# CompVis/behavior-driven-video-synthesis

Hardware: AMD Instinct MI355X
Metric: frames/sec VUnet 256x256 bs=16 fwd+bwd (higher is better)
Workload: dtype f32 (operands scaled by a power of two and split into 2 fp16 terms, 3 partial products on fp16 MFMA, fp32 accumulate; weight gradients and uncovered layers: 3 bf16 terms / 6 products, fp32-input MFMA, fp32 VALU); 1 GPU; Human3.6m shape_and_pose_net VunetAlter 256x256 per-GPU bs=16 fwd+bwd, VGG19 perceptual + KL loss, fused Adam, dropout 0.05, regressor side loop off, seeded-synthetic VGG19 weights, rasterised synthetic stickmen; global_batch=16, parallelism=dp1, conv_precision=h2, hip_streams=4, hip_graph=True, graph_settle_steps=7, rccl_world_size=1, dp_backend=none

## Files before the change

behavior_driven_video_synthesis_amd/csrc/pointwise.hip:

```cpp
#include "common.h"

static inline dim3 ew_grid(int64_t n, int per_thread = 1) {
  int64_t b = (n + 256ll * per_thread - 1) / (256ll * per_thread);
  if (b > 2048) b = 2048;
  if (b < 1) b = 1;
  return dim3((unsigned)b);
}

#define EW_LOOP(i, n) \
  for (int64_t i = (int64_t)blockIdx.x * blockDim.x + threadIdx.x; i < (n); i += (int64_t)gridDim.x * blockDim.x)

__device__ __forceinline__ float block_sum_256(float v, float* red) {
  v = wave_sum(v);
  __syncthreads();
  if ((threadIdx.x & 63) == 0) red[threadIdx.x >> 6] = v;
  __syncthreads();
  return red[0] + red[1] + red[2] + red[3];
}

__device__ __forceinline__ float pool2_max(float e0, float e1, float e2, float e3) {
  const float m = fmaxf(fmaxf(e0, e1), fmaxf(e2, e3));
  return e3 != e3 ? e3 : (e2 != e2 ? e2 : (e1 != e1 ? e1 : (e0 != e0 ? e0 : m)));
}
__device__ __forceinline__ int pool2_route(float e0, float e1, float e2, float e3) {
// ... 339 lines not shown
__global__ void maxpool2_fwd_kernel(const float* __restrict__ x, float* __restrict__ y, int H, int W, int64_t n) {
  const int Ho = H >> 1, Wo = W >> 1;
  EW_LOOP(o, n) {
    const int ow = (int)(o % Wo);
    const int64_t t = o / Wo;
    const int oh = (int)(t % Ho);
    const int64_t nc = t / Ho;
    const float* r0 = x + (nc * H + 2 * oh) * W + 2 * ow;
    const float2 a = *reinterpret_cast<const float2*>(r0);
    const float2 b = *reinterpret_cast<const float2*>(r0 + W);
    y[o] = pool2_max(a.x, a.y, b.x, b.y);
  }
}
__global__ void maxpool2_bwd_kernel(const float* __restrict__ x, const float* __restrict__ y,
                                    const float* __restrict__ dy, float* __restrict__ dx, int H, int W, int64_t n,
                                    int relu_mask) {
  const int Ho = H >> 1, Wo = W >> 1;
  EW_LOOP(o, n) {
    const int ow = (int)(o % Wo);
    const int64_t t = o / Wo;
    const int oh = (int)(t % Ho);
    const int64_t nc = t / Ho;
    const int64_t i0 = (nc * H + 2 * oh) * W + 2 * ow;
    const float m = y[o];
    const float g = (relu_mask && m <= 0.f) ? 0.f : dy[o];
    const float2 a = *reinterpret_cast<const float2*>(x + i0);
    const float2 b = *reinterpret_cast<const float2*>(x + i0 + W);
    const int k = pool2_route(a.x, a.y, b.x, b.y);
    *reinterpret_cast<float2*>(dx + i0) = make_float2(k == 0 ? g : 0.f, k == 1 ? g : 0.f);
    *reinterpret_cast<float2*>(dx + i0 + W) = make_float2(k == 2 ? g : 0.f, k == 3 ? g : 0.f);
  }
}
extern "C" int vunet_maxpool2_fwd(const float* x, float* y, int32_t NC, int32_t H, int32_t W, void* st) {
  if (!x || !y || (H & 1) || (W & 1)) return VUNET_ERR_ARG;
  const int64_t n = (int64_t)NC * (H / 2) * (W / 2);
  VUNET_LAUNCH(maxpool2_fwd_kernel, ew_grid(n), dim3(256), 0, (hipStream_t)st, x, y, H, W, n);
  return vunet_check_launch();
}
__global__ void l1_pool_bwd_kernel(const float* __restrict__ a, const float* __restrict__ b, const float* __restrict__ dyp,
                                   float* __restrict__ db, float gs, const float* __restrict__ gout, int H, int W, int64_t n,
                                   float* __restrict__ amax_out, int relu_mask) {
  if (gout) gs *= gout[0];
  const int Ho = H >> 1, Wo = W >> 1;
  float vmax = 0.f;
  EW_LOOP(o, n) {
    const int ow = (int)(o % Wo);
    const int64_t t = o / Wo;
    const int oh = (int)(t % Ho);
    const int64_t nc = t / Ho;
    const int64_t i0 = (nc * H + 2 * oh) * W + 2 * ow;
    const float2 b0 = *reinterpret_cast<const float2*>(b + i0), b1 = *reinterpret_cast<const float2*>(b + i0 + W);
    const float2 a0 = *reinterpret_cast<const float2*>(a + i0), a1 = *reinterpret_cast<const float2*>(a + i0 + W);
    const float g = dyp ? dyp[o] : 0.f;
    const int k = pool2_route(b0.x, b0.y, b1.x, b1.y);
    const float bv[4] = {b0.x, b0.y, b1.x, b1.y}, av[4] = {a0.x, a0.y, a1.x, a1.y};
    float v[4];
#pragma unroll
    for (int e = 0; e < 4; ++e) {
      const float d = bv[e] - av[e];
      float r = (k == e ? g : 0.f) + (d > 0.f ? gs : (d < 0.f ? -gs : 0.f));
      if (relu_mask && bv[e] <= 0.f) r = 0.f;
      v[e] = r;
      vmax = fmaxf(vmax, fabsf(r));
    }
    *reinterpret_cast<float2*>(db + i0) = make_float2(v[0], v[1]);
    *reinterpret_cast<float2*>(db + i0 + W) = make_float2(v[2], v[3]);
  }
  if (amax_out) {
    const float m_ = wave_max(vmax);
    if ((threadIdx.x & 63) == 0)
      atomicMax(reinterpret_cast<unsigned*>(amax_out) + ((blockIdx.x * 4u + (threadIdx.x >> 6)) & 511u), __float_as_uint(m_));
  }
}
extern "C" int vunet_l1_pool_bwd(const float* a, const float* b, const float* dy_pool, float* db, float gscale,
                                 const float* gout, int32_t NC, int32_t H, int32_t W, float* amax_out, int32_t relu_mask,
                                 void* st) {
  if (!a || !b || !db || (H & 1) || (W & 1)) return VUNET_ERR_ARG;
  const int64_t n = (int64_t)NC * (H / 2) * (W / 2);
  VUNET_LAUNCH(l1_pool_bwd_kernel, ew_grid(n), dim3(256), 0, (hipStream_t)st, a, b, dy_pool, db, gscale, gout, H, W, n,
               amax_out, (int)relu_mask);
  return vunet_check_launch();
}

static int maxpool2_bwd(const float* x, const float* y, const float* dy, float* dx, int32_t NC, int32_t H, int32_t W,
                        int relu_mask, void* st) {
  if (!x || !y || !dy || !dx || (H & 1) || (W & 1)) return VUNET_ERR_ARG;
  const int64_t n = (int64_t)NC * (H / 2) * (W / 2);
  VUNET_LAUNCH(maxpool2_bwd_kernel, ew_grid(n), dim3(256), 0, (hipStream_t)st, x, y, dy, dx, H, W, n, relu_mask);
  return vunet_check_launch();
}
extern "C" int vunet_maxpool2_bwd(const float* x, const float* y, const float* dy, float* dx, int32_t NC, int32_t H,
                                  int32_t W, void* st) {
  return maxpool2_bwd(x, y, dy, dx, NC, H, W, 0, st);
}
extern "C" int vunet_maxpool2_bwd_relu(const float* x, const float* y, const float* dy, float* dx, int32_t NC, int32_t H,
                                       int32_t W, void* st) {
  return maxpool2_bwd(x, y, dy, dx, NC, H, W, 1, st);
}

__global__ __launch_bounds__(256) void instnorm_fwd_kernel(const float* __restrict__ x, float* __restrict__ y,
                                                           float* __restrict__ stats, int HW, float eps) {
  __shared__ float red[4];
  const float* xr = x + (size_t)blockIdx.x * HW;
  float* yr = y + (size_t)blockIdx.x * HW;
  float s = 0.f;
  for (int i = threadIdx.x; i < HW; i += 256) s += xr[i];
  const float mean = block_sum_256(s, red) / (float)HW;
  float v = 0.f;
  for (int i = threadIdx.x; i < HW; i += 256) { const float d = xr[i] - mean; v += d * d; }
  const float var = block_sum_256(v, red) / (float)HW;
  const float rstd = rsqrtf(var + eps);
  for (int i = threadIdx.x; i < HW; i += 256) yr[i] = (xr[i] - mean) * rstd;
  if (threadIdx.x == 0) { stats[2 * blockIdx.x] = mean; stats[2 * blockIdx.x + 1] = rstd; }
}
__global__ __launch_bounds__(256) void instnorm_bwd_kernel(const float* __restrict__ y, const float* __restrict__ dy,
                                                           const float* __restrict__ stats, float* __restrict__ dx,
                                                           int HW) {
  __shared__ float red[4];
  const size_t o = (size_t)blockIdx.x * HW;
  float s1 = 0.f, s2 = 0.f;
  for (int i = threadIdx.x; i < HW; i += 256) { const float g = dy[o + i]; s1 += g; s2 += g * y[o + i]; }
  const float m1 = block_sum_256(s1, red) / (float)HW;
  const float m2 = block_sum_256(s2, red) / (float)HW;
  const float rstd = stats[2 * blockIdx.x + 1];
  for (int i = threadIdx.x; i < HW; i += 256) dx[o + i] = rstd * (dy[o + i] - m1 - y[o + i] * m2);
}
extern "C" int vunet_instnorm_fwd(const float* x, float* y, float* stats, int32_t NC, int32_t HW, float eps, void* st) {
  if (!x || !y || !stats || NC <= 0 || HW <= 0) return VUNET_ERR_ARG;
  VUNET_LAUNCH(instnorm_fwd_kernel, dim3(NC), dim3(256), 0, (hipStream_t)st, x, y, stats, HW, eps);
  return vunet_check_launch();
}
extern "C" int vunet_instnorm_bwd(const float* y, const float* dy, const float* stats, float* dx, int32_t NC,
                                  int32_t HW, void* st) {
  if (!y || !dy || !stats || !dx) return VUNET_ERR_ARG;
  VUNET_LAUNCH(instnorm_bwd_kernel, dim3(NC), dim3(256), 0, (hipStream_t)st, y, dy, stats, dx, HW);
  return vunet_check_launch();
}

const uint32_t* g_vunet_drop_step = nullptr;

extern "C" int vunet_set_dropout_step(const uint32_t* step_dev) {
  g_vunet_drop_step = step_dev;
  return VUNET_OK;
}

int g_vunet_tune[16] = {0};

extern "C" int vunet_set_tuning(int32_t key, int32_t value) {
  if (key < 0 || key >= VUNET_TUNE_COUNT) return VUNET_ERR_ARG;
  g_vunet_tune[key] = value;
  return VUNET_OK;
}

__global__ void adam_kernel(float* __restrict__ p, const float* __restrict__ g, float* __restrict__ m,
                            float* __restrict__ v, int64_t n, float step_size, float b1, float b2, float eps,
                            float wd, float inv_sqrt_bc2, float gscale) {
  EW_LOOP(i, n) {
    float gi = g[i] * gscale;
    const float pi = p[i];
    if (wd != 0.f) gi += wd * pi;
    const float mi = b1 * m[i] + (1.f - b1) * gi;
    const float vi = b2 * v[i] + (1.f - b2) * gi * gi;
    m[i] = mi;
    v[i] = vi;
    const float denom = sqrtf(vi) * inv_sqrt_bc2 + eps;
    p[i] = pi - step_size * (mi / denom);
  }
}
extern "C" int vunet_adam_step(float* param, const float* grad, float* exp_avg, float* exp_avg_sq, int64_t n, float lr,
                               float beta1, float beta2, float eps, float weight_decay, int32_t step,
                               float grad_scale, void* st) {
  if (!param || !grad || !exp_avg || !exp_avg_sq || step < 1) return VUNET_ERR_ARG;
  const double bc1 = 1.0 - pow((double)beta1, (double)step);
  const double bc2 = 1.0 - pow((double)beta2, (double)step);
  VUNET_LAUNCH(adam_kernel, ew_grid(n), dim3(256), 0, (hipStream_t)st, param, grad, exp_avg, exp_avg_sq, n,
                     (float)(lr / bc1), beta1, beta2, eps, weight_decay, (float)(1.0 / sqrt(bc2)), grad_scale);
  return vunet_check_launch();
}

__global__ void adam_dev_kernel(float* __restrict__ p, const float* __restrict__ g, float* __restrict__ m,
                                float* __restrict__ v, int64_t n, const double* __restrict__ lr,
                                const int64_t* __restrict__ step, float b1, float b2, float eps, float wd, float gscale) {
  const double t = (double)*step;
  const double bc1 = 1.0 - pow((double)b1, t), bc2 = 1.0 - pow((double)b2, t);
  const float step_size = (float)((double)(float)*lr / bc1), inv_sqrt_bc2 = (float)(1.0 / sqrt(bc2));
  EW_LOOP(i, n) {
    float gi = g[i] * gscale;
    const float pi = p[i];
    if (wd != 0.f) gi += wd * pi;
    const float mi = b1 * m[i] + (1.f - b1) * gi;
    const float vi = b2 * v[i] + (1.f - b2) * gi * gi;
    m[i] = mi;
    v[i] = vi;
    const float denom = sqrtf(vi) * inv_sqrt_bc2 + eps;
    p[i] = pi - step_size * (mi / denom);
  }
}
extern "C" int vunet_adam_step_dev(float* param, const float* grad, float* exp_avg, float* exp_avg_sq, int64_t n,
                                   const double* lr_dev, float beta1, float beta2, float eps, float weight_decay,
                                   const int64_t* step_dev, float grad_scale, void* st) {
  if (!param || !grad || !exp_avg || !exp_avg_sq || !lr_dev || !step_dev) return VUNET_ERR_ARG;
  VUNET_LAUNCH(adam_dev_kernel, ew_grid(n), dim3(256), 0, (hipStream_t)st, param, grad, exp_avg, exp_avg_sq, n, lr_dev,
               step_dev, beta1, beta2, eps, weight_decay, grad_scale);
  return vunet_check_launch();
}

__global__ __launch_bounds__(256) void absmax_partials_kernel(const float* __restrict__ x1, int64_t n1,
                                                              const float* __restrict__ x2, int64_t n2,
                                                              float* __restrict__ out) {
  __shared__ float red[4];
  const bool second = blockIdx.x >= 512;
  const float* __restrict__ x = second ? x2 : x1;
  const int64_t n = second ? n2 : n1;
  const int b = second ? blockIdx.x - 512 : blockIdx.x;
  float m = 0.f;
  if (x) {
    const int64_t n4 = ((reinterpret_cast<uintptr_t>(x) & 15) == 0) ? n >> 2 : 0;
    const float4* __restrict__ x4 = reinterpret_cast<const float4*>(x);
    for (int64_t i = (int64_t)b * 256 + threadIdx.x; i < n4; i += 512 * 256) {
      const float4 v = x4[i];
      m = fmaxf(fmaxf(m, fmaxf(fabsf(v.x), fabsf(v.y))), fmaxf(fabsf(v.z), fabsf(v.w)));
    }
    for (int64_t i = 4 * n4 + (int64_t)b * 256 + threadIdx.x; i < n; i += 512 * 256) m = fmaxf(m, fabsf(x[i]));
  }
  m = wave_max(m);
  if ((threadIdx.x & 63) == 0) red[threadIdx.x >> 6] = m;
  __syncthreads();
  if (threadIdx.x == 0) out[blockIdx.x] = fmaxf(fmaxf(red[0], red[1]), fmaxf(red[2], red[3]));
}
extern "C" int vunet_absmax_partials(const float* x1, int64_t n1, const float* x2, int64_t n2, float* out, void* st) {
  if (!x1 || !out || n1 < 0 || n2 < 0) return VUNET_ERR_ARG;
  VUNET_LAUNCH(absmax_partials_kernel, dim3(1024), dim3(256), 0, (hipStream_t)st, x1, n1, x2, x2 ? n2 : 0, out);
  return vunet_check_launch();
}

__global__ void dropout_mask_kernel(float* mask, int64_t n, uint32_t thresh, uint32_t seed, const uint32_t* step) {
  if (step) seed += (*step) * VUNET_DROP_STEP_MUL;
  EW_LOOP(i, n) mask[i] = vunet_hash_u32((uint32_t)i + seed) >= thresh ? 1.f : 0.f;
}
extern "C" int vunet_dropout_mask(float* mask, int64_t n, float p, uint32_t seed, void* st) {
  if (!mask) return VUNET_ERR_ARG;
  const InAct a = make_inact(ACT_NONE, 0.f, p, seed);
  VUNET_LAUNCH(dropout_mask_kernel, ew_grid(n), dim3(256), 0, (hipStream_t)st, mask, n, a.thresh, seed, a.step);
  return vunet_check_launch();
}
__global__ void u8_to_unit_kernel(const uint8_t* in, float* out, int64_t n) {
  EW_LOOP(i, n) out[i] = ((float)in[i] / 255.0f) * 2.0f - 1.0f;
}
extern "C" int vunet_u8_to_unit(const uint8_t* in, float* out, int64_t n, void* st) {
  if (!in || !out) return VUNET_ERR_ARG;
  VUNET_LAUNCH(u8_to_unit_kernel, ew_grid(n), dim3(256), 0, (hipStream_t)st, in, out, n);
  return vunet_check_launch();
}

__device__ __forceinline__ void bil2_src(int o, int n, int& i0, int& i1, float& l) {
  const int i = o >> 1;
  if (o & 1) { i0 = i; l = 0.25f; }
  else if (i == 0) { i0 = 0; l = 0.f; }
  else { i0 = i - 1; l = 0.75f; }
  i1 = i0 + 1 < n ? i0 + 1 : n - 1;
}

__global__ void bilinear2x_fwd_kernel(const float* __restrict__ x, float* __restrict__ y, int64_t NC, int H, int W) {
  const int H2 = 2 * H, W2 = 2 * W;
  EW_LOOP(o, NC * H2 * W2) {
    const int ox = (int)(o % W2);
    const int64_t t = o / W2;
    const int oy = (int)(t % H2);
    const float* p = x + (t / H2) * H * W;
    int y0, y1, x0, x1;
    float ly, lx;
    bil2_src(oy, H, y0, y1, ly);
    bil2_src(ox, W, x0, x1, lx);
    const float top = (1.f - lx) * p[y0 * W + x0] + lx * p[y0 * W + x1];
    const float bot = (1.f - lx) * p[y1 * W + x0] + lx * p[y1 * W + x1];
    y[o] = (1.f - ly) * top + ly * bot;
  }
}

__device__ __forceinline__ void bil2_adj(int i, int n, int o[4], float w[4]) {
  o[0] = 2 * i - 1; w[0] = i >= 1 ? 0.25f : 0.f;
  o[1] = 2 * i;     w[1] = i == 0 ? 1.f : 0.75f;
  o[2] = 2 * i + 1; w[2] = i == n - 1 ? 1.f : 0.75f;
  o[3] = 2 * i + 2; w[3] = i <= n - 2 ? 0.25f : 0.f;
  if (o[0] < 0) o[0] = 0;
  if (o[3] > 2 * n - 1) o[3] = 2 * n - 1;
}

__global__ void bilinear2x_bwd_kernel(const float* __restrict__ dy, float* __restrict__ dx, int64_t NC, int H, int W) {
  const int W2 = 2 * W;
  EW_LOOP(e, NC * H * W) {
    const int ix = (int)(e % W);
    const int64_t t = e / W;
    const int iy = (int)(t % H);
    const float* p = dy + (t / H) * 4 * H * W;
    int oy[4], ox[4];
    float wy[4], wx[4];
    bil2_adj(iy, H, oy, wy);
    bil2_adj(ix, W, ox, wx);
    float s = 0.f;
#pragma unroll
    for (int a = 0; a < 4; ++a) {
      float r = 0.f;
#pragma unroll
      for (int b = 0; b < 4; ++b) r += wx[b] * p[oy[a] * W2 + ox[b]];
      s += wy[a] * r;
    }
    dx[e] = s;
  }
}

extern "C" int vunet_upsample_bilinear2x_fwd(const float* x, float* y, int64_t NC, int32_t H, int32_t W, void* st) {
  if (!x || !y || NC < 1 || H < 1 || W < 1) return VUNET_ERR_ARG;
  VUNET_LAUNCH(bilinear2x_fwd_kernel, ew_grid(NC * 4 * H * W), dim3(256), 0, (hipStream_t)st, x, y, NC, H, W);
  return vunet_check_launch();
}

extern "C" int vunet_upsample_bilinear2x_bwd(const float* dy, float* dx, int64_t NC, int32_t H, int32_t W, void* st) {
  if (!dy || !dx || NC < 1 || H < 1 || W < 1) return VUNET_ERR_ARG;
  VUNET_LAUNCH(bilinear2x_bwd_kernel, ew_grid(NC * H * W), dim3(256), 0, (hipStream_t)st, dy, dx, NC, H, W);
  return vunet_check_launch();
}

extern "C" int vunet_abi_version(void) { return 12; }

__global__ void crop_window_kernel(const float* __restrict__ x, float* __restrict__ y, int planes, int H, int W, int P,
                                   const int32_t* __restrict__ off, int bwd) {
  const int oy = off[0], ox = off[1];
  const int64_t n = (int64_t)planes * P * P;
  EW_LOOP(i, n) {
    const int j = (int)(i % P), r = (int)((i / P) % P);
    const int64_t pl = i / ((int64_t)P * P);
    const int64_t src = (pl * H + (oy + r)) * W + (ox + j);
    if (bwd) y[src] = x[i];
    else y[i] = x[src];
  }
}
extern "C" int vunet_crop_window(const float* x, float* y, int32_t planes, int32_t H, int32_t W, int32_t P, const int32_t* off,
                                 void* st) {
  if (!x || !y || !off || planes < 1 || P < 1 || P > H || P > W) return VUNET_ERR_ARG;
  VUNET_LAUNCH(crop_window_kernel, ew_grid((int64_t)planes * P * P), dim3(256), 0, (hipStream_t)st, x, y, planes, H, W, P, off, 0);
  return vunet_check_launch();
}
extern "C" int vunet_crop_window_bwd(const float* dy, float* dx, int32_t planes, int32_t H, int32_t W, int32_t P,
                                     const int32_t* off, void* st) {
  if (!dy || !dx || !off || planes < 1 || P < 1 || P > H || P > W) return VUNET_ERR_ARG;
  VUNET_LAUNCH(crop_window_kernel, ew_grid((int64_t)planes * P * P), dim3(256), 0, (hipStream_t)st, dy, dx, planes, H, W, P, off, 1);
  return vunet_check_launch();
}

struct LossTermPtrs {
  const float* t[VUNET_LOSS_MAX_TERMS];
};
__global__ void total_loss_kernel(LossTermPtrs a, int n, const float* __restrict__ kl, const float* __restrict__ gamma,
                                  float gamma_const, float ll_weight, int use_kl, float* __restrict__ loss,
// ... 112 lines not shown
```

behavior_driven_video_synthesis_amd/csrc/weightnorm.hip:

```cpp
#include "common.h"
#include "split_h2.h"

#define X6_SLAB_UNITS 576

struct WnArgs {
  vunet_wn_desc d;
  const float *v, *g, *bias, *gamma, *beta;
  float *wt_f, *wt_d, *scale, *shift, *invnorm;
  uint4 *wx_f, *wx_d;
  float* wmax;
  int T, Ctot, C1p, C2p, Kf, Mpad_f, Coutp2, Kd, Mpad_d;
};

__host__ __device__ __forceinline__ int x6_mtiles(int m) { return (((m + 31) / 32 + 1) + 1) & ~1; }

__device__ __forceinline__ uint32_t wn_pack2(float a, float b) {
  typedef __bf16 bf2 __attribute__((ext_vector_type(2)));
  bf2 p;
  p[0] = (__bf16)a;
  p[1] = (__bf16)b;
  return __builtin_bit_cast(uint32_t, p);
}

__device__ __forceinline__ void wn_split2(float a, float b, uint32_t& h, uint32_t& m, uint32_t& l) {
// ... 281 lines not shown
  const uint32_t nd = a.wt_d ? (uint32_t)a.Kd * (uint32_t)a.Mpad_d : 0u;
  const int T = a.T;
  for (uint32_t i = (uint32_t)start; i < nf + nd; i += (uint32_t)stride) {
    if (i < nf) {
      const int krow = (int)(i / (uint32_t)a.Mpad_f), m = (int)(i - (uint32_t)krow * (uint32_t)a.Mpad_f);
      int tap, c, cg;
      bool ok;
      const int k1 = T * a.C1p;
      if (krow < k1) { tap = krow / a.C1p; c = krow - tap * a.C1p; ok = c < a.d.C1; cg = c; }
      else { const int r = krow - k1; tap = r / a.C2p; c = r - tap * a.C2p; ok = c < a.d.C2; cg = a.d.C1 + c; }
      float w = 0.f;
      if (ok && m < a.d.Cout) w = a.scale[m] * a.v[((size_t)m * a.Ctot + cg) * T + tap];
      a.wt_f[i] = w;
    } else {
      const uint32_t e = i - nf;
      const int row = (int)(e / (uint32_t)a.Mpad_d), ci = (int)(e - (uint32_t)row * (uint32_t)a.Mpad_d);
      const int tap = row / a.Coutp2, co = row - tap * a.Coutp2;
      float w = 0.f;
      if (co < a.d.Cout && ci < a.Ctot) w = a.scale[co] * a.v[((size_t)co * a.Ctot + ci) * T + tap];
      a.wt_d[e] = w;
    }
  }
}

__global__ __launch_bounds__(64) void wn_scale_multi_kernel(const WnItemDev* __restrict__ items) {
  const WnItemDev& it = items[blockIdx.y];
  if ((int)blockIdx.x >= it.d.Cout) return;
  wn_scale_body(item_args(it), blockIdx.x, threadIdx.x);
}

constexpr int WN_TILE_LD = 145;

__device__ __forceinline__ bool wn_tiled_ok(const WnArgs& a) {
  return a.T == 9 && a.d.split == 2 && a.wx_f != nullptr && a.d.C1 % 16 == 0 && a.d.C2 % 16 == 0;
}

__device__ __forceinline__ void wn_pack_tile(const WnArgs& a, int mtile, int ch, float* tile) {
  const int tid = threadIdx.x;
  const int nch1 = a.d.C1 / 16;
  const bool second = ch >= nch1;
  const int cg0 = second ? a.d.C1 + (ch - nch1) * 16 : ch * 16;
  const int m0 = mtile * 32;
  const int ew = wn_layer_exp(a);
  const float sw = h2_pow2(ew);
  for (int e = tid; e < 32 * 144; e += 256) {
    const int r = e / 144, k = e - r * 144;
    const int co = m0 + r;
    tile[r * WN_TILE_LD + k] = co < a.d.Cout ? a.scale[co] * a.v[((size_t)co * a.Ctot + cg0) * 9 + k] : 0.f;
  }
  __syncthreads();
  {
    const int cl0 = second ? (ch - nch1) * 16 : ch * 16;
    const int krow0 = second ? 9 * a.C1p : 0, Cp = second ? a.C2p : a.C1p;
    for (int e = tid; e < 32 * 144; e += 256) {
      const int m = e & 31, q = e >> 5;
      const int ci = q & 15, tap = q >> 4;
      a.wt_f[(size_t)(krow0 + tap * Cp + cl0 + ci) * a.Mpad_f + m0 + m] = tile[m * WN_TILE_LD + ci * 9 + tap];
    }
  }
  if (a.wt_d) {
    for (int e = tid; e < 32 * 144; e += 256) {
      const int ci = e & 15, q = e >> 4;
      const int r = q & 31, tap = q >> 5;
      const int co = m0 + r;
      if (co < a.Coutp2) a.wt_d[(size_t)(tap * a.Coutp2 + co) * a.Mpad_d + cg0 + ci] = tile[r * WN_TILE_LD + ci * 9 + tap];
    }
  }
  {
    uint4* const out = a.wx_f + 1;
    const int mtp = x6_mtiles(a.d.Cout);
    if (mtile == 0 && ch == 0 && tid == 0) a.wx_f[0] = make_uint4((uint32_t)ew, 0u, 0u, 0u);
    for (int e = tid; e < 9 * 2 * 32; e += 256) {
      const int j = e & 31, half = (e >> 5) & 1, tap = e >> 6;
      const int kh = tap / 3, kw = tap - 3 * kh;
      float w[8];
#pragma unroll
      for (int c = 0; c < 8; ++c) w[c] = tile[j * WN_TILE_LD + (half * 8 + c) * 9 + tap] * sw;
      uint4 ph, pl;
      h2_split2(w[0], w[1], ph.x, pl.x);
      h2_split2(w[2], w[3], ph.y, pl.y);
      h2_split2(w[4], w[5], ph.z, pl.z);
      h2_split2(w[6], w[7], ph.w, pl.w);
      const size_t base = ((((size_t)(ch * 3 + kh) * mtp + mtile) * 3 + kw) * 2) * 64 + half * 32 + j;
      out[base] = ph;
      out[base + 64] = pl;
    }
  }
  if (a.wx_d) {
    uint4* const out = a.wx_d + 1;
    const int mtp = x6_mtiles(a.Ctot);
    if (mtile == 0 && ch == 0 && tid == 0) a.wx_d[0] = make_uint4((uint32_t)ew, 0u, 0u, 0u);
    for (int e = tid; e < 2 * 9 * 2 * 16; e += 256) {
      const int ci = e & 15, half = (e >> 4) & 1;
      const int q = e >> 5;
      const int tap = q % 9, chl = q / 9;
      const int chd = 2 * mtile + chl;
      if (chd * 16 >= a.d.Cout) continue;
      const int kh = tap / 3, kw = tap - 3 * kh;
      float w[8];
#pragma unroll
      for (int c = 0; c < 8; ++c) w[c] = tile[(chl * 16 + half * 8 + c) * WN_TILE_LD + ci * 9 + tap] * sw;
      uint4 ph, pl;
      h2_split2(w[0], w[1], ph.x, pl.x);
      h2_split2(w[2], w[3], ph.y, pl.y);
      h2_split2(w[4], w[5], ph.z, pl.z);
      h2_split2(w[6], w[7], ph.w, pl.w);
      const int cgt = cg0 + ci;
      const size_t base = ((((size_t)(chd * 3 + kh) * mtp + (cgt >> 5)) * 3 + kw) * 2) * 64 + half * 32 + (cgt & 31);
      out[base] = ph;
      out[base + 64] = pl;
    }
  }
}

__global__ __launch_bounds__(256) void wn_pack_multi_kernel(const WnItemDev* __restrict__ items) {
  __shared__ float tile[32 * WN_TILE_LD];
  const WnArgs a = item_args(items[blockIdx.y]);
  if (wn_tiled_ok(a)) {
    const int ntm = (a.d.Cout + 31) / 32, nch = a.Ctot / 16;
    for (int t = blockIdx.x; t < ntm * nch; t += gridDim.x) {
      wn_pack_tile(a, t % ntm, t / ntm, tile);
      __syncthreads();
    }
    return;
  }
  const size_t n = (size_t)a.Kf * a.Mpad_f + (a.wt_d ? (size_t)a.Kd * a.Mpad_d : 0);
  size_t nb = (n + 1023) / 1024;
  if (nb > gridDim.x) nb = gridDim.x;
  if (nb < 1) nb = 1;
  if (blockIdx.x >= nb) return;
  wn_pack_body(a, (size_t)blockIdx.x * 256 + threadIdx.x, nb * 256);
  wn_pack_split_body(a, (size_t)blockIdx.x * 256 + threadIdx.x, nb * 256);
}

extern "C" int vunet_weightnorm_fwd_multi(const vunet_wn_item* items_dev, int32_t n_items, int32_t max_cout,
                                          void* stream) {
  if (!items_dev || n_items < 1 || max_cout < 1) return VUNET_ERR_ARG;
  static_assert(sizeof(WnItemDev) == sizeof(vunet_wn_item), "vunet_wn_item layout");
  const WnItemDev* items = reinterpret_cast<const WnItemDev*>(items_dev);
  hipStream_t st = (hipStream_t)stream;
  VUNET_LAUNCH(wn_scale_multi_kernel, dim3((unsigned)max_cout, (unsigned)n_items), dim3(64), 0, st, items);
  VUNET_LAUNCH(wn_pack_multi_kernel, dim3(512, (unsigned)n_items), dim3(256), 0, st, items);
  return vunet_check_launch();
}

struct WnBwdArgs {
  vunet_wn_desc d;
  const float *slabs, *dshift, *v, *g, *bias, *gamma, *invnorm;
  float *dv, *dg, *dbias, *dgamma, *dbeta;
  float *dwred, *dsred;
  int nsplit, T, Ctot, Coutp, accumulate;
};

__device__ __forceinline__ void wn_slab_reduce_body(const WnBwdArgs& a, int block, float (*part)[64]) {
  const int lane = threadIdx.x & 63, wave = threadIdx.x >> 6;
  const int K = a.T * a.Ctot;
  const int kchunks = (K + 63) / 64;
  const int co = block / kchunks, kc = block - co * kchunks;
  const int k = kc * 64 + lane;
  float s = 0.f;
  if (k < K) {
    const float* p = a.slabs + (size_t)co * K + k;
    const size_t stride = (size_t)a.Coutp * K;
#pragma unroll 8
    for (int sl = wave; sl < a.nsplit; sl += 4) s += p[(size_t)sl * stride];
  }
  part[wave][lane] = s;
  __syncthreads();
  if (wave == 0 && k < K) {
    const float tot = (part[0][lane] + part[1][lane]) + (part[2][lane] + part[3][lane]);
    const int tap = k / a.Ctot, ci = k - tap * a.Ctot;
    a.dwred[(size_t)co * K + ci * a.T + tap] = tot;
  }
  if (kc == 0 && wave == 1) {
    float t = 0.f;
    for (int sl = lane; sl < a.nsplit; sl += 64) t += a.dshift[(size_t)sl * a.Coutp + co];
    t = wave_sum(t);
    if (lane == 0) a.dsred[co] = t;
  }
}

__global__ __launch_bounds__(256) void wn_slab_reduce_kernel(const WnBwdArgs a) {
  __shared__ float part[4][64];
  wn_slab_reduce_body(a, blockIdx.x, part);
}

__device__ __forceinline__ void wn_bwd_body(const WnBwdArgs& a, int co, float* red) {
  const int tid = threadIdx.x;
  const int K = a.T * a.Ctot;
  const float* vr = a.v + (size_t)co * K;
  const float* dwr = a.dwred + (size_t)co * K;
  float dot = 0.f;
  for (int k = tid; k < K; k += 256) dot += dwr[k] * vr[k];
  dot = wave_sum(dot);
  if ((tid & 63) == 0) red[tid >> 6] = dot;
  __syncthreads();
  const float D = red[0] + red[1] + red[2] + red[3];
  const float dsh = a.dsred[co];
#define WN_OLD(ptr) (a.accumulate ? (ptr)[co] : 0.f)

  const int kind = a.d.kind;
  const float invn = kind == 1 ? 1.f : a.invnorm[co];
  const float gm = (kind != 1 && a.gamma) ? a.gamma[co] : 1.f;
  const float gg = kind == 0 ? a.g[co] : 1.f;
  const float b = a.bias ? a.bias[co] : 0.f;
  if (tid == 0) {
    if (kind == 1) {
      if (a.dbias) a.dbias[co] = WN_OLD(a.dbias) + dsh;
    } else {
      if (a.dgamma) a.dgamma[co] = WN_OLD(a.dgamma) + (gg * invn * D + b * dsh);
      if (a.dbeta) a.dbeta[co] = WN_OLD(a.dbeta) + dsh;
      if (a.dbias) a.dbias[co] = WN_OLD(a.dbias) + gm * dsh;
      if (a.dg && kind == 0) a.dg[co] = WN_OLD(a.dg) + gm * invn * D;
    }
  }
  if (a.dv) {
    const float c0 = gm * gg * invn, c1 = invn * invn * D;
    float* dvr = a.dv + (size_t)co * K;
    for (int k = tid; k < K; k += 256) {
      const float dw = dwr[k];
      const float val = kind == 1 ? dw : c0 * (dw - c1 * vr[k]);
      dvr[k] = a.accumulate ? dvr[k] + val : val;
    }
  }
#undef WN_OLD
}

__global__ __launch_bounds__(256) void wn_bwd_kernel(const WnBwdArgs a) {
  __shared__ float red[4];
  wn_bwd_body(a, blockIdx.x, red);
}

struct WnBwdItemDev {
  const float *slabs, *dshift, *v, *g, *bias, *gamma, *invnorm;
  float *dv, *dg, *dbias, *dgamma, *dbeta;
  float* workspace;
  vunet_wn_desc d;
  int32_t nsplit, accumulate;
};

__device__ __forceinline__ WnBwdArgs bwd_item_args(const WnBwdItemDev& it) {
  WnBwdArgs a;
  a.d = it.d;
  a.slabs = it.slabs; a.dshift = it.dshift; a.v = it.v; a.g = it.g; a.bias = it.bias; a.gamma = it.gamma;
  a.invnorm = it.invnorm;
  a.dv = it.dv; a.dg = it.dg; a.dbias = it.dbias; a.dgamma = it.dgamma; a.dbeta = it.dbeta;
  a.nsplit = it.nsplit;
  a.T = it.d.KH * it.d.KW;
  a.Ctot = it.d.C1 + it.d.C2;
  a.Coutp = (it.d.Cout + 31) / 32 * 32;
  a.accumulate = it.accumulate;
  a.dwred = it.workspace;
  a.dsred = it.workspace + (size_t)it.d.Cout * a.T * a.Ctot;
  return a;
}

__global__ __launch_bounds__(256) void wn_slab_reduce_multi_kernel(const WnBwdItemDev* __restrict__ items) {
  __shared__ float part[4][64];
  const WnBwdArgs a = bwd_item_args(items[blockIdx.y]);
  const int nb = a.d.Cout * ((a.T * a.Ctot + 63) / 64);
  for (int b = blockIdx.x; b < nb; b += gridDim.x) {
    wn_slab_reduce_body(a, b, part);
    __syncthreads();
  }
}

__global__ __launch_bounds__(256) void wn_bwd_multi_kernel(const WnBwdItemDev* __restrict__ items) {
  __shared__ float red[4];
  const WnBwdItemDev& it = items[blockIdx.y];
  if ((int)blockIdx.x >= it.d.Cout) return;
  wn_bwd_body(bwd_item_args(it), blockIdx.x, red);
}

extern "C" int vunet_weightnorm_bwd_multi(const vunet_wn_bwd_item* items_dev, int32_t n_items, int32_t max_cout,
                                          int32_t max_reduce_blocks, void* stream) {
  if (!items_dev || n_items < 1 || max_cout < 1 || max_reduce_blocks < 1) return VUNET_ERR_ARG;
  static_assert(sizeof(WnBwdItemDev) == sizeof(vunet_wn_bwd_item), "vunet_wn_bwd_item layout");
  const WnBwdItemDev* items = reinterpret_cast<const WnBwdItemDev*>(items_dev);
  hipStream_t st = (hipStream_t)stream;
  int gx = 4096 / n_items;
  if (gx < 16) gx = 16;
  if (gx > max_reduce_blocks) gx = max_reduce_blocks;
  VUNET_LAUNCH(wn_slab_reduce_multi_kernel, dim3((unsigned)gx, (unsigned)n_items), dim3(256), 0, st, items);
  VUNET_LAUNCH(wn_bwd_multi_kernel, dim3((unsigned)max_cout, (unsigned)n_items), dim3(256), 0, st, items);
  return vunet_check_launch();
}

extern "C" int vunet_weightnorm_bwd(const vunet_wn_desc* d, const float* slabs, const float* dshift, int32_t nsplit,
                                    const float* v, const float* g, const float* bias, const float* gamma,
                                    const float* invnorm, float* dv, float* dg, float* dbias, float* dgamma,
                                    float* dbeta, float* workspace, int32_t accumulate, void* stream) {
  if (!d || !slabs || !dshift || !v || !workspace || nsplit < 1) return VUNET_ERR_ARG;
  if (d->kind != 1 && !invnorm) return VUNET_ERR_ARG;
  if (d->kind == 0 && !g) return VUNET_ERR_ARG;
  WnBwdArgs a;
  a.d = *d;
  a.slabs = slabs; a.dshift = dshift; a.v = v; a.g = g; a.bias = bias; a.gamma = gamma; a.invnorm = invnorm;
  a.dv = dv; a.dg = dg; a.dbias = dbias; a.dgamma = dgamma; a.dbeta = dbeta;
  a.nsplit = nsplit;
  a.T = d->KH * d->KW;
  a.Ctot = d->C1 + d->C2;
  a.Coutp = (d->Cout + 31) / 32 * 32;
  a.accumulate = accumulate;
  const int K = a.T * a.Ctot;
  a.dwred = workspace;
  a.dsred = workspace + (size_t)d->Cout * K;
  const int kchunks = (K + 63) / 64;
  VUNET_LAUNCH(wn_slab_reduce_kernel, dim3((unsigned)(d->Cout * kchunks)), dim3(256), 0, (hipStream_t)stream, a);
  VUNET_LAUNCH(wn_bwd_kernel, dim3(d->Cout), dim3(256), 0, (hipStream_t)stream, a);
  return vunet_check_launch();
}
```

Before: 795.3 frames/s.

## Vectorise Adam update and restructure weight-norm slab reduction per wave

Adam now processes float4 chunks when all four buffers share alignment, with a scalar head/tail path and a grid sized for four elements per thread. It keeps explicit fma placement to control rounding. The weight-norm backward slab reduction is reworked so each wave owns a unit, chosen among three layouts by split count and alignment, with float4 loads and deeper unrolling. The dshift reduction moves into its own wave-strided loop, and the shared-memory cross-wave combine is gone. The aim is to cut memory-bound time in the optimizer and gradient reduction, at the cost of more code paths and possible rounding differences.

```diff
diff --git a/behavior_driven_video_synthesis_amd/csrc/pointwise.hip b/behavior_driven_video_synthesis_amd/csrc/pointwise.hip
--- a/behavior_driven_video_synthesis_amd/csrc/pointwise.hip
+++ b/behavior_driven_video_synthesis_amd/csrc/pointwise.hip
@@ -515,20 +515,55 @@
   return VUNET_OK;
 }
 
+__device__ __forceinline__ void adam_update(float& p, float g, float& m, float& v, float step_size, float b1, float b2,
+                                            float eps, float wd, float inv_sqrt_bc2, float gscale) {
+#pragma clang fp contract(off)
+  float gi = g * gscale;
+  const float pi = p;
+  if (wd != 0.f) gi = gi + wd * pi;
+  const float mi = __builtin_fmaf(1.f - b1, gi, b1 * m);
+  const float vi = b2 * v + ((1.f - b2) * gi) * gi;
+  m = mi;
+  v = vi;
+  const float denom = __builtin_fmaf(sqrtf(vi), inv_sqrt_bc2, eps);
+  p = __builtin_fmaf(-step_size, mi / denom, pi);
+}
+__device__ __forceinline__ void adam_body(float* __restrict__ p, const float* __restrict__ g, float* __restrict__ m,
+                                          float* __restrict__ v, int64_t n, float step_size, float b1, float b2, float eps,
+                                          float wd, float inv_sqrt_bc2, float gscale) {
+  const unsigned mis = (unsigned)(reinterpret_cast<uintptr_t>(p) >> 2) & 3u;
+  const bool alike = ((reinterpret_cast<uintptr_t>(p) ^ reinterpret_cast<uintptr_t>(g)) & 15) == 0 &&
+                     ((reinterpret_cast<uintptr_t>(p) ^ reinterpret_cast<uintptr_t>(m)) & 15) == 0 &&
+                     ((reinterpret_cast<uintptr_t>(p) ^ reinterpret_cast<uintptr_t>(v)) & 15) == 0 &&
+                     (reinterpret_cast<uintptr_t>(p) & 3) == 0;
+  int64_t head = alike ? (int64_t)((4u - mis) & 3u) : n;
+  if (head > n) head = n;
+  const int64_t n4 = (n - head) >> 2;
+  float4* __restrict__ p4 = reinterpret_cast<float4*>(p + head);
+  const float4* __restrict__ g4 = reinterpret_cast<const float4*>(g + head);
+  float4* __restrict__ m4 = reinterpret_cast<float4*>(m + head);
+  float4* __restrict__ v4 = reinterpret_cast<float4*>(v + head);
+  EW_LOOP(i, n4) {
+    float4 pv = p4[i], mv = m4[i], vv = v4[i];
+    const float4 gv = g4[i];
+    adam_update(pv.x, gv.x, mv.x, vv.x, step_size, b1, b2, eps, wd, inv_sqrt_bc2, gscale);
+    adam_update(pv.y, gv.y, mv.y, vv.y, step_size, b1, b2, eps, wd, inv_sqrt_bc2, gscale);
+    adam_update(pv.z, gv.z, mv.z, vv.z, step_size, b1, b2, eps, wd, inv_sqrt_bc2, gscale);
+    adam_update(pv.w, gv.w, mv.w, vv.w, step_size, b1, b2, eps, wd, inv_sqrt_bc2, gscale);
+    m4[i] = mv;
+    v4[i] = vv;
+    p4[i] = pv;
+  }
+  const int64_t tail0 = head + 4 * n4, nrest = head + (n - tail0);
+  EW_LOOP(r, nrest) {
+    const int64_t i = r < head ? r : tail0 + (r - head);
+    adam_update(p[i], g[i], m[i], v[i], step_size, b1, b2, eps, wd, inv_sqrt_bc2, gscale);
+  }
+}
 __global__ void adam_kernel(float* __restrict__ p, const float* __restrict__ g, float* __restrict__ m,
                             float* __restrict__ v, int64_t n, float step_size, float b1, float b2, float eps,
                             float wd, float inv_sqrt_bc2, float gscale) {
-  EW_LOOP(i, n) {
-    float gi = g[i] * gscale;
-    const float pi = p[i];
-    if (wd != 0.f) gi += wd * pi;
-    const float mi = b1 * m[i] + (1.f - b1) * gi;
-    const float vi = b2 * v[i] + (1.f - b2) * gi * gi;
-    m[i] = mi;
-    v[i] = vi;
-    const float denom = sqrtf(vi) * inv_sqrt_bc2 + eps;
-    p[i] = pi - step_size * (mi / denom);
-  }
+  adam_body(p, g, m, v, n, step_size, b1, b2, eps, wd, inv_sqrt_bc2, gscale);
 }
 extern "C" int vunet_adam_step(float* param, const float* grad, float* exp_avg, float* exp_avg_sq, int64_t n, float lr,
                                float beta1, float beta2, float eps, float weight_decay, int32_t step,
@@ -536,7 +571,7 @@
   if (!param || !grad || !exp_avg || !exp_avg_sq || step < 1) return VUNET_ERR_ARG;
   const double bc1 = 1.0 - pow((double)beta1, (double)step);
   const double bc2 = 1.0 - pow((double)beta2, (double)step);
-  VUNET_LAUNCH(adam_kernel, ew_grid(n), dim3(256), 0, (hipStream_t)st, param, grad, exp_avg, exp_avg_sq, n,
+  VUNET_LAUNCH(adam_kernel, ew_grid(n, 4), dim3(256), 0, (hipStream_t)st, param, grad, exp_avg, exp_avg_sq, n,
                      (float)(lr / bc1), beta1, beta2, eps, weight_decay, (float)(1.0 / sqrt(bc2)), grad_scale);
   return vunet_check_launch();
 }
@@ -547,23 +582,13 @@
   const double t = (double)*step;
   const double bc1 = 1.0 - pow((double)b1, t), bc2 = 1.0 - pow((double)b2, t);
   const float step_size = (float)((double)(float)*lr / bc1), inv_sqrt_bc2 = (float)(1.0 / sqrt(bc2));
-  EW_LOOP(i, n) {
-    float gi = g[i] * gscale;
-    const float pi = p[i];
-    if (wd != 0.f) gi += wd * pi;
-    const float mi = b1 * m[i] + (1.f - b1) * gi;
-    const float vi = b2 * v[i] + (1.f - b2) * gi * gi;
-    m[i] = mi;
-    v[i] = vi;
-    const float denom = sqrtf(vi) * inv_sqrt_bc2 + eps;
-    p[i] = pi - step_size * (mi / denom);
-  }
+  adam_body(p, g, m, v, n, step_size, b1, b2, eps, wd, inv_sqrt_bc2, gscale);
 }
 extern "C" int vunet_adam_step_dev(float* param, const float* grad, float* exp_avg, float* exp_avg_sq, int64_t n,
                                    const double* lr_dev, float beta1, float beta2, float eps, float weight_decay,
                                    const int64_t* step_dev, float grad_scale, void* st) {
   if (!param || !grad || !exp_avg || !exp_avg_sq || !lr_dev || !step_dev) return VUNET_ERR_ARG;
-  VUNET_LAUNCH(adam_dev_kernel, ew_grid(n), dim3(256), 0, (hipStream_t)st, param, grad, exp_avg, exp_avg_sq, n, lr_dev,
+  VUNET_LAUNCH(adam_dev_kernel, ew_grid(n, 4), dim3(256), 0, (hipStream_t)st, param, grad, exp_avg, exp_avg_sq, n, lr_dev,
                step_dev, beta1, beta2, eps, weight_decay, grad_scale);
   return vunet_check_launch();
 }
diff --git a/behavior_driven_video_synthesis_amd/csrc/weightnorm.hip b/behavior_driven_video_synthesis_amd/csrc/weightnorm.hip
--- a/behavior_driven_video_synthesis_amd/csrc/weightnorm.hip
+++ b/behavior_driven_video_synthesis_amd/csrc/weightnorm.hip
@@ -457,37 +457,166 @@
   int nsplit, T, Ctot, Coutp, accumulate;
 };
 
-__device__ __forceinline__ void wn_slab_reduce_body(const WnBwdArgs& a, int block, float (*part)[64]) {
-  const int lane = threadIdx.x & 63, wave = threadIdx.x >> 6;
-  const int K = a.T * a.Ctot;
-  const int kchunks = (K + 63) / 64;
-  const int co = block / kchunks, kc = block - co * kchunks;
-  const int k = kc * 64 + lane;
-  float s = 0.f;
-  if (k < K) {
-    const float* p = a.slabs + (size_t)co * K + k;
-    const size_t stride = (size_t)a.Coutp * K;
+#define WN_SPLIT_FROM 65
+#define WN_SINGLE_FROM 512
+
+__device__ __forceinline__ void slab_add4(float4& w, const float4& x) {
+  w.x += x.x; w.y += x.y; w.z += x.z; w.w += x.w;
+}
+
+template <int LAYOUT, bool VEC>
+__device__ __forceinline__ void wn_slab_reduce_unit(const WnBwdArgs& a, int unit) {
+  constexpr bool SPLIT = LAYOUT != 0;
+  constexpr int GW = LAYOUT == 2 ? 1 : 4;
+  constexpr int EPW = SPLIT ? 16 * GW : 256;
+  const int lane = threadIdx.x & 63;
+  const int K = a.T * a.Ctot, total = a.d.Cout * K;
+  const int e0 = unit * EPW + GW * (SPLIT ? lane >> 2 : lane);
+  const size_t stride = (size_t)a.Coutp * K;
+  const float* const p0 = a.slabs + e0;
+  auto ld = [&](int sl) -> float4 {
+    const float* p = p0 + (size_t)sl * stride;
+    float4 x = make_float4(0.f, 0.f, 0.f, 0.f);
+    if (VEC) {
+      if (e0 < total) x = *reinterpret_cast<const float4*>(p);
+    } else {
+      if (e0 < total) x.x = p[0];
+      if (e0 + 1 < total) x.y = p[1];
+      if (e0 + 2 < total) x.z = p[2];
+      if (e0 + 3 < total) x.w = p[3];
+    }
+    return x;
+  };
+  if constexpr (!SPLIT) {
+    float4 w[4];
+#pragma unroll
+    for (int i = 0; i < 4; ++i) w[i] = make_float4(0.f, 0.f, 0.f, 0.f);
+    int sl = 0;
+    for (; sl + 16 <= a.nsplit; sl += 16) {
+      float4 x[16];
+#pragma unroll
+      for (int i = 0; i < 16; ++i) x[i] = ld(sl + i);
+#pragma unroll
+      for (int i = 0; i < 16; ++i) slab_add4(w[i & 3], x[i]);
+    }
+    for (; sl + 4 <= a.nsplit; sl += 4) {
+      float4 x[4];
+#pragma unroll
+      for (int i = 0; i < 4; ++i) x[i] = ld(sl + i);
+#pragma unroll
+      for (int i = 0; i < 4; ++i) slab_add4(w[i], x[i]);
+    }
+    {
+      const int rem = a.nsplit - sl;
+      float4 x[3];
+#pragma unroll
+      for (int i = 0; i < 3; ++i)
+        if (i < rem) x[i] = ld(sl + i);
+#pragma unroll
+      for (int i = 0; i < 3; ++i)
+        if (i < rem) slab_add4(w[i], x[i]);
+    }
+    const float tot[4] = {(w[0].x + w[1].x) + (w[2].x + w[3].x), (w[0].y + w[1].y) + (w[2].y + w[3].y),
+                          (w[0].z + w[1].z) + (w[2].z + w[3].z), (w[0].w + w[1].w) + (w[2].w + w[3].w)};
+    if (e0 < total) {
+      int co = e0 / K;
+      const int k = e0 - co * K;
+      int tap = k / a.Ctot, ci = k - tap * a.Ctot;
+#pragma unroll
+      for (int i = 0; i < 4; ++i) {
+        if (e0 + i < total) a.dwred[(size_t)co * K + ci * a.T + tap] = tot[i];
+        if (++ci == a.Ctot) {
+          ci = 0;
+          if (++tap == a.T) {
+            tap = 0;
+            ++co;
+          }
+        }
+      }
+    }
+  } else {
+    const int i = lane & 3;
+    constexpr int UN = GW == 4 ? 16 : 32;
+    float w[GW];
+#pragma unroll
+    for (int c = 0; c < GW; ++c) w[c] = 0.f;
+    auto ldg = [&](int sl, float (&x)[GW]) {
+      if constexpr (GW == 4) {
+        const float4 v = ld(sl);
+        x[0] = v.x; x[1] = v.y; x[2] = v.z; x[3] = v.w;
+      } else {
+        x[0] = e0 < total ? p0[(size_t)sl * stride] : 0.f;
+      }
+    };
+    int sl = i;
+    for (; sl + 4 * (UN - 1) < a.nsplit; sl += 4 * UN) {
+      float x[UN][GW];
+#pragma unroll
+      for (int q = 0; q < UN; ++q) ldg(sl + 4 * q, x[q]);
+#pragma unroll
+      for (int q = 0; q < UN; ++q)
+#pragma unroll
+        for (int c = 0; c < GW; ++c) w[c] += x[q][c];
+    }
+    for (; sl < a.nsplit; sl += 4) {
+      float x[GW];
+      ldg(sl, x);
+#pragma unroll
+      for (int c = 0; c < GW; ++c) w[c] += x[c];
+    }
+#pragma unroll
+    for (int c = 0; c < GW; ++c) {
+      w[c] = w[c] + __shfl_xor(w[c], 1, 64);
+      w[c] = w[c] + __shfl_xor(w[c], 2, 64);
+    }
+    const int e = e0 + (GW == 4 ? i : 0);
+    if (e < total && (GW == 4 || i == 0)) {
+      const int co = e / K, k = e - co * K;
+      const int tap = k / a.Ctot, ci = k - tap * a.Ctot;
+      float t = w[0];
+      if constexpr (GW == 4) t = i == 0 ? w[0] : i == 1 ? w[1] : i == 2 ? w[2] : w[3];
+      a.dwred[(size_t)co * K + ci * a.T + tap] = t;
+    }
+  }
+}
+
+__device__ __forceinline__ void wn_dshift_reduce(const WnBwdArgs& a, int wave_id, int nwaves) {
+  const int lane = threadIdx.x & 63;
+  for (int co = wave_id; co < a.d.Cout; co += nwaves) {
+    const float* const p = a.dshift + co;
+    float t = 0.f;
 #pragma unroll 8
-    for (int sl = wave; sl < a.nsplit; sl += 4) s += p[(size_t)sl * stride];
-  }
-  part[wave][lane] = s;
-  __syncthreads();
-  if (wave == 0 && k < K) {
-    const float tot = (part[0][lane] + part[1][lane]) + (part[2][lane] + part[3][lane]);
-    const int tap = k / a.Ctot, ci = k - tap * a.Ctot;
-    a.dwred[(size_t)co * K + ci * a.T + tap] = tot;
-  }
-  if (kc == 0 && wave == 1) {
-    float t = 0.f;
-    for (int sl = lane; sl < a.nsplit; sl += 64) t += a.dshift[(size_t)sl * a.Coutp + co];
+    for (int sl = lane; sl < a.nsplit; sl += 64) t += p[(size_t)sl * a.Coutp];
     t = wave_sum(t);
     if (lane == 0) a.dsred[co] = t;
   }
 }
 
+static __host__ __device__ __forceinline__ bool wn_slab_reduce_vec(const float* slabs, int K) {
+  return (K & 3) == 0 && (reinterpret_cast<uintptr_t>(slabs) & 15) == 0;
+}
+static __host__ __device__ __forceinline__ int wn_slab_reduce_layout(const float* slabs, int K, int nsplit) {
+  if (nsplit < WN_SPLIT_FROM) return 0;
+  return wn_slab_reduce_vec(slabs, K) && nsplit < WN_SINGLE_FROM ? 1 : 2;
+}
+static __host__ __device__ __forceinline__ int wn_slab_reduce_units(const float* slabs, int cout, int K, int nsplit) {
+  const int layout = wn_slab_reduce_layout(slabs, K, nsplit), epw = layout == 0 ? 256 : layout == 1 ? 64 : 16;
+  return (cout * K + epw - 1) / epw;
+}
+
+__device__ __forceinline__ void wn_slab_reduce_body(const WnBwdArgs& a, int unit) {
+  const bool vec = wn_slab_reduce_vec(a.slabs, a.T * a.Ctot);
+  const int layout = wn_slab_reduce_layout(a.slabs, a.T * a.Ctot, a.nsplit);
+  if (layout == 2) wn_slab_reduce_unit<2, false>(a, unit);
+  else if (layout == 1) wn_slab_reduce_unit<1, true>(a, unit);
+  else if (vec) wn_slab_reduce_unit<0, true>(a, unit);
+  else wn_slab_reduce_unit<0, false>(a, unit);
+}
+
 __global__ __launch_bounds__(256) void wn_slab_reduce_kernel(const WnBwdArgs a) {
-  __shared__ float part[4][64];
-  wn_slab_reduce_body(a, blockIdx.x, part);
+  const int unit = blockIdx.x * 4 + (threadIdx.x >> 6);
+  wn_dshift_reduce(a, unit, gridDim.x * 4);
+  if (unit < wn_slab_reduce_units(a.slabs, a.d.Cout, a.T * a.Ctot, a.nsplit)) wn_slab_reduce_body(a, unit);
 }
 
 __device__ __forceinline__ void wn_bwd_body(const WnBwdArgs& a, int co, float* red) {
@@ -561,13 +690,10 @@
 }
 
 __global__ __launch_bounds__(256) void wn_slab_reduce_multi_kernel(const WnBwdItemDev* __restrict__ items) {
-  __shared__ float part[4][64];
   const WnBwdArgs a = bwd_item_args(items[blockIdx.y]);
-  const int nb = a.d.Cout * ((a.T * a.Ctot + 63) / 64);
-  for (int b = blockIdx.x; b < nb; b += gridDim.x) {
-    wn_slab_reduce_body(a, b, part);
-    __syncthreads();
-  }
+  const int nu = wn_slab_reduce_units(a.slabs, a.d.Cout, a.T * a.Ctot, a.nsplit);
+  wn_dshift_reduce(a, blockIdx.x * 4 + (threadIdx.x >> 6), gridDim.x * 4);
+  for (int u = blockIdx.x * 4 + (threadIdx.x >> 6); u < nu; u += gridDim.x * 4) wn_slab_reduce_body(a, u);
 }
 
 __global__ __launch_bounds__(256) void wn_bwd_multi_kernel(const WnBwdItemDev* __restrict__ items) {
@@ -610,8 +736,8 @@
   const int K = a.T * a.Ctot;
   a.dwred = workspace;
   a.dsred = workspace + (size_t)d->Cout * K;
-  const int kchunks = (K + 63) / 64;
-  VUNET_LAUNCH(wn_slab_reduce_kernel, dim3((unsigned)(d->Cout * kchunks)), dim3(256), 0, (hipStream_t)stream, a);
+  const int units = wn_slab_reduce_units(slabs, d->Cout, K, nsplit);
+  VUNET_LAUNCH(wn_slab_reduce_kernel, dim3((unsigned)((units + 3) / 4)), dim3(256), 0, (hipStream_t)stream, a);
   VUNET_LAUNCH(wn_bwd_kernel, dim3(d->Cout), dim3(256), 0, (hipStream_t)stream, a);
   return vunet_check_launch();
 }
```

New measurement: 799.6 frames/s, median of 3. No clear change (+0.5%).
